# Strong-AI-Lab/ct-vae

Hardware: AMD Instinct MI355X
Metric: images/sec/GPU fwd+bwd, 64×64×3 bs=64; recon+KL vs CPU ref (higher is better)
Workload: dtype f32; 1 GPU; VanillaVAE 64x64x3 train step fwd+loss+bwd+Adam (configs/vae.yaml shapes at the batch BASELINE.json's metric names, bs=64, on one MI355X; BASELINE.json configs[1..4] are the `configs` entries); per_gpu_batch=64, global_batch=64, latent_dim=128, parallelism=single, hipgraph=True, allreduce_overlap=False

## Files before the change

### ct-vae_amd/csrc/pair.hpp

```cpp
#pragma once
#include <functional>
#include <vector>

#include "finish.hpp"
#include "tapgemm.hpp"
#include "wgrad_fast.hpp"

namespace ctvae {

struct PairCtx {
  bool haveA = false, haveB = false;
  long dgrad_wgs = 0;
  int dgrad_chunks = 0;
  TapGemmArgs A;
  unsigned gxA = 0, gyA = 0, gzA = 0;
  double flopsA = 0, bytesA = 0;
  WgradArgs B;
  int lgQw = -1, lgQhw = -1, lgC = -1;
  unsigned gxB = 0, gyB = 0;
  double flopsB = 0, bytesB = 0;
  bool haveSK = false, haveRed = false;
  SplitKJob sk;
  ReduceJob j1, j2;
  int nb1 = 0, nb2 = 0, accumulate = 0;
  double bytesSK = 0, bytesRed = 0;
  bool haveBF = false;
  BnFinJob bf;
  std::vector<std::function<int()>> later;
};

PairCtx*& pair_ctx();
int pair_flush(PairCtx& c, hipStream_t st);
int launch_wgrad_fast_recorded(const PairCtx& c, hipStream_t st);
int launch_finish_recorded(const PairCtx& c, hipStream_t st);
int launch_splitk_recorded(const PairCtx& c, hipStream_t st);
int launch_bn_bwd_finalize_job(const BnFinJob& j, hipStream_t st);

}
```

### ct-vae_amd/csrc/tapgemm_fast.hip

```cpp
#include <type_traits>

#include "prof.hpp"
#include "pair.hpp"
#include "tapgemm.hpp"
#include "wgrad_fast.hpp"

namespace ctvae {

typedef unsigned int u32x4 __attribute__((ext_vector_type(4)));
constexpr unsigned kOOB = 0x80000000u;

__device__ __forceinline__ f32x4 buf_load4(__amdgpu_buffer_rsrc_t r, unsigned voff, unsigned soff) {
  return __builtin_bit_cast(f32x4, __builtin_amdgcn_raw_buffer_load_b128(r, (int)voff, (int)soff, 0));
}
__device__ __forceinline__ float buf_load1(__amdgpu_buffer_rsrc_t r, unsigned voff) {
  return __builtin_bit_cast(float, __builtin_amdgcn_raw_buffer_load_b32(r, (int)voff, 0, 0));
}
__device__ __forceinline__ void buf_store1(__amdgpu_buffer_rsrc_t r, unsigned voff, float v) {
  __builtin_amdgcn_raw_buffer_store_b32(__builtin_bit_cast(unsigned, v), r, (int)voff, 0, 0);
}
__device__ __forceinline__ __amdgpu_buffer_rsrc_t make_rsrc(const void* p, long bytes) {
  return __builtin_amdgcn_make_buffer_rsrc(const_cast<void*>(p), 0, (int)bytes, 0x00020000);
}

// ... 3 lines not shown
__device__ long long g_loop[4 * 8192];
#define LOOPT(var) const long long var = clock64()
#define LOOPACC(i, a, b) loopt_[i] += (b) - (a)
#define LOOPDECL long long loopt_[4] = {0, 0, 0, 0}
#define LOOPOUT do { if (threadIdx.x == 0 && blockIdx.z == 0) for (int q_ = 0; q_ < 4; ++q_) g_loop[((blockIdx.y * gridDim.x + blockIdx.x) & 8191) * 4 + q_] = loopt_[q_]; } while (0)
extern "C" int ctvae_debug_loop_read(long long* out, int n) { return (int)hipMemcpyFromSymbol(out, HIP_SYMBOL(g_loop), (size_t)n * 8); }
extern "C" int ctvae_debug_phase_read(unsigned long long* out, int n) {
  return (int)hipMemcpyFromSymbol(out, HIP_SYMBOL(g_phase), (size_t)n * 8);
}
extern "C" int ctvae_debug_wphase_read(unsigned long long* out, int n) {
  return (int)hipMemcpyFromSymbol(out, HIP_SYMBOL(g_wphase), (size_t)n * 8);
}
#else
#define PHASE(i) do {} while (0)
#define LOOPT(var) do {} while (0)
#define LOOPACC(i, a, b) do {} while (0)
#define LOOPDECL do {} while (0)
#define LOOPOUT do {} while (0)
#endif

template <int WM, int WN, int TM, int TN, bool WT, int PF, bool XF = false, int PD = 1>
__global__ __launch_bounds__(256) void tapgemm_fast_kernel(const TapGemmArgs a) {
  __shared__ __attribute__((aligned(16))) float sAbuf[(PF == 3 ? 2 : 1) * (WM * TM * 32) * LDK];
  __shared__ __attribute__((aligned(16))) float sBbuf[(PF == 3 ? 2 : 1) * (WT ? (WN * TN * 32) * LDK : KC * (WN * TN * 32))];
  __shared__ __attribute__((aligned(16))) int sOut[WM * TM * 32];
  PHASE(0);
  int k_cls_rot, k_mtiles, k_ntiles;
  kernarg_warm_get<sizeof(TapGemmArgs), offsetof(TapGemmArgs, cls_rot), offsetof(TapGemmArgs, mtiles), offsetof(TapGemmArgs, ntiles)>(
      k_cls_rot, k_mtiles, k_ntiles);
  const int vbx = blockIdx.x, vby = blockIdx.y, vbz = blockIdx.z, vgx = k_mtiles * k_ntiles;
#include "tapgemm_fast_body.inc"
}

template <bool XFB, int PDA = 1>
__global__ __launch_bounds__(256) void conv_bwd_pair_kernel(const TapGemmArgs a, const WgradArgs w, int lgQw, int lgQhw, int lgC,
                                                            int nA, int gxA, int gyA, int gxB, int gyB) {
  __shared__ __attribute__((aligned(16))) float sAbuf[2 * 64 * LDK];
  __shared__ __attribute__((aligned(16))) float sBbuf[2 * 64 * LDK];
  __shared__ __attribute__((aligned(16))) int sOut[64];
  __shared__ unsigned sPix[2][MC];
  __shared__ unsigned sMsk[2][MC];
  __shared__ unsigned sOutB[2][MC];
  static_assert(2 * 64 * LDK >= MC * 64, "chunk buffers of the weight-gradient kernel fit");
  constexpr int kOffW = (sizeof(TapGemmArgs) + 7) / 8 * 8, kOffI = kOffW + sizeof(WgradArgs);
  static_assert(alignof(TapGemmArgs) == 8 && alignof(WgradArgs) == 8 && sizeof(WgradArgs) % 8 == 0, "kernel-argument layout");
  int k_nA, k_gxA, k_gyA;
  kernarg_warm_get<kOffI + 8 * 4, kOffI + 12, kOffI + 16, kOffI + 20>(k_nA, k_gxA, k_gyA);
  const int L = blockIdx.x;
  if (L < k_nA) {
    constexpr int WM = 2, WN = 2, TM = 1, TN = 1, PF = 3;
    constexpr bool WT = true, XF = false;
    constexpr int PD = PDA;
    const int vbx = L % k_gxA, vr = L / k_gxA, vby = vr % k_gyA, vbz = vr / k_gyA, vgx = k_gxA;
    const int k_cls_rot = a.cls_rot, k_ntiles = a.ntiles;
#include "tapgemm_fast_body.inc"
  } else {
    const int Lb = L - k_nA;
    wgrad_fast_body<2, 2, 1, 1, XFB>(w, lgQw, lgQhw, lgC, sAbuf, sBbuf, sPix, sMsk, sOutB, Lb % gxB, Lb / gxB, gxB, gyB);
  }
}

template <int WM, int WN, int TM, int TN>
static int launch_fast_cfg(const TapGemmArgs& a, int pf, hipStream_t st) {
  constexpr int BM = WM * TM * 32, BN = WN * TN * 32;
  TapGemmArgs args = a;
  args.mtiles = ceil_div(a.Mc, BM);
  args.ntiles = ceil_div(a.N, BN);
  const bool wt = a.g.wT != 0;
  dim3 grid(args.mtiles * args.ntiles, a.g.ncls, a.splitk > 1 ? a.splitk : 1), block(256);
  for (int c = 0; c < kMaxCls; ++c) args.cls_order[c] = c;
  args.cls_rot = 0;
  if (a.g.ncls == 4) {
    int idx[4] = {0, 1, 2, 3};
    for (int i = 1; i < 4; ++i)
      for (int j = i; j > 0 && a.g.ntaps[idx[j]] < a.g.ntaps[idx[j - 1]]; --j) { const int t = idx[j]; idx[j] = idx[j - 1]; idx[j - 1] = t; }
    const long total = (long)grid.x * grid.y * grid.z;
    if (total <= 1024) {
      args.cls_order[0] = idx[0]; args.cls_order[1] = idx[1]; args.cls_order[2] = idx[3]; args.cls_order[3] = idx[2];
      args.cls_rot = grid.z > 1 ? 1 : 0;
    }
  }
  for (int i = 0; i < kMaxCls; ++i) {
    const int c = args.cls_order[i];
    args.ntaps_l[i] = a.g.ntaps[c];
    for (int t = 0; t < kMaxTaps; ++t) args.taps_l[i][t] = a.g.taps[c][t];
  }
  constexpr bool deep = false;
  char name[160];
  snprintf(name, sizeof name, "tapgemm_fast_kernel<%d,%d,%d,%d,%s,%d%s>", WM, WN, TM, TN, wt ? "true" : "false", pf,
           (!wt && a.xf_scale != nullptr) ? ",true" : (deep ? ",false,4" : ""));
  double macs = 0;
  for (int c = 0; c < a.g.ncls; ++c) macs += (double)a.Mc * a.N * a.g.ntaps[c] * a.g.gC;
  if constexpr (WM == 2 && WN == 2 && TM == 1 && TN == 1) {
    PairCtx* pc = pair_ctx();
    if (pc != nullptr && wt && pf == 3 && !pc->haveA) {
      pc->haveA = true;
      pc->A = args;
      pc->gxA = grid.x; pc->gyA = grid.y; pc->gzA = grid.z;
      pc->flopsA = 2.0 * macs;
      pc->bytesA = 4.0 * ((double)a.g.B * a.g.gH * a.g.gW * a.g.gC + (double)a.g.B * a.g.sH * a.g.sW * a.g.sC);
      return 0;
    }
  }
  if (prof_detailed()) {
    size_t l = strlen(name);
    snprintf(name + l, sizeof name - l, " M=%dx%d N=%d C=%d taps=%d sk=%d", a.g.ncls, a.Mc, a.N, a.g.gC, a.g.ntaps[a.g.ncls - 1],
             a.splitk);
  }
  const double bytes = 4.0 * ((double)a.g.B * a.g.gH * a.g.gW * a.g.gC + (double)a.g.B * a.g.sH * a.g.sW * a.g.sC);
  ProfScope ps(name, st, 2.0 * macs, bytes);
  if (!wt && a.xf_scale != nullptr) {
    if (pf == 3) hipLaunchKernelGGL((tapgemm_fast_kernel<WM, WN, TM, TN, false, 3, true>), grid, block, 0, st, args);
    else hipLaunchKernelGGL((tapgemm_fast_kernel<WM, WN, TM, TN, false, 0, true>), grid, block, 0, st, args);
  } else if (!wt) {
    if (pf == 3) hipLaunchKernelGGL((tapgemm_fast_kernel<WM, WN, TM, TN, false, 3>), grid, block, 0, st, args);
    else hipLaunchKernelGGL((tapgemm_fast_kernel<WM, WN, TM, TN, false, 0>), grid, block, 0, st, args);
  } else {
    if (pf == 3) hipLaunchKernelGGL((tapgemm_fast_kernel<WM, WN, TM, TN, true, 3>), grid, block, 0, st, args);
    else hipLaunchKernelGGL((tapgemm_fast_kernel<WM, WN, TM, TN, true, 0>), grid, block, 0, st, args);
  }
  CTVAE_LAUNCH_CHECK();
  return 0;
}

PairCtx*& pair_ctx() {
  static thread_local PairCtx* ctx = nullptr;
  return ctx;
}

int pair_flush(PairCtx& c, hipStream_t st) {
  if (c.haveA && c.haveB) {
    const unsigned nA = c.gxA * c.gyA * c.gzA, nB = c.gxB * c.gyB;
    ProfScope ps("conv_bwd_pair_kernel", st, c.flopsA + c.flopsB, c.bytesA + c.bytesB);
#define CTVAE_PAIR(XFB_, PD_)                                                                                                  \
  hipLaunchKernelGGL((conv_bwd_pair_kernel<XFB_, PD_>), dim3(nA + nB), dim3(256), 0, st, c.A, c.B, c.lgQw, c.lgQhw, c.lgC, (int)nA, \
                     (int)c.gxA, (int)c.gyA, (int)c.gxB, (int)c.gyB)
    if (c.B.xf_scale != nullptr) CTVAE_PAIR(true, 1);
    else CTVAE_PAIR(false, 1);
#undef CTVAE_PAIR
    CTVAE_LAUNCH_CHECK();
  } else if (c.haveA) {
    ProfScope ps("tapgemm_fast_kernel<2,2,1,1,true,3>", st, c.flopsA, c.bytesA);
    hipLaunchKernelGGL((tapgemm_fast_kernel<2, 2, 1, 1, true, 3>), dim3(c.gxA, c.gyA, c.gzA), dim3(256), 0, st, c.A);
    CTVAE_LAUNCH_CHECK();
  } else if (c.haveB) {
    const int rc = launch_wgrad_fast_recorded(c, st);
    if (rc) return rc;
  }
  if (c.haveRed || (c.haveSK && c.haveBF)) {
    const int rc = launch_finish_recorded(c, st);
    if (rc) return rc;
  } else {
    if (c.haveSK) {
      const int rc = launch_splitk_recorded(c, st);
      if (rc) return rc;
    }
    if (c.haveBF) {
      const int rc = launch_bn_bwd_finalize_job(c.bf, st);
      if (rc) return rc;
    }
  }
  for (auto& f : c.later) {
    const int rc = f();
    if (rc) return rc;
  }
  return 0;
}

int launch_tapgemm_fast(const TapGemmArgs& a, const TapGemmPlan& plan, int pf, hipStream_t st) {
  if (plan.BN == 32) return launch_fast_cfg<4, 1, 1, 1>(a, pf, st);
  if (plan.BM == 128) return launch_fast_cfg<2, 2, 2, 1>(a, pf, st);
  return launch_fast_cfg<2, 2, 1, 1>(a, pf, st);
}

}
```

### ct-vae_amd/csrc/wgrad.hip

```cpp
#include "common.hpp"
#include "prof.hpp"
#include "finish.hpp"
#include "pair.hpp"
#include "wgrad_fast.hpp"

namespace ctvae {


template <int WK, int WN, bool XVEC, bool DVEC>
__global__ __launch_bounds__(256) void wgrad_kernel(const WgradArgs a) {
  kernarg_warm<sizeof(WgradArgs)>();
  constexpr int KT = WK * 32, NT = WN * 32;
  static_assert(WK * WN == 4, "4 waves");
  __shared__ __attribute__((aligned(16))) float sXbuf[MC * KT];
  __shared__ __attribute__((aligned(16))) float sDbuf[MC * NT];
  __shared__ int sRowPix[2][MC];
  __shared__ int sRowYX[2][MC];
  __shared__ int sRowOut[2][MC];

  const ConvGeom& g = a.g;
  const int tid = threadIdx.x, lane = tid & 63, wave = tid >> 6;
  const int wk = wave / WN, wn = wave % WN;
  const int li = lane & 31, lh = lane >> 5;
  int split = blockIdx.y, xtile = blockIdx.x;
  {
    const int T = gridDim.x, L = blockIdx.y * T + blockIdx.x, full = (gridDim.y >> 3) * 8 * T;
    if (L < full) {
      const int grp = L / (8 * T), r = L - grp * 8 * T;
      split = grp * 8 + (r & 7);
      xtile = r >> 3;
    }
  }
  const int ktg = xtile / a.ntiles, nt = xtile - ktg * a.ntiles;
  int cls = 0;
#pragma unroll
  for (int c = 1; c < kMaxCls; ++c)
    if (c < g.ncls && ktg >= a.ktile_start[c]) cls = c;
  const int kt0 = (ktg - a.ktile_start[cls]) * KT;
  const int n0 = nt * NT;
  const int gC = g.gC;
  const int Ktot = g.ntaps[cls] * gC;
  const int N = a.N;

  const int cbeg = split * a.chunks_per_split;
  const int nchunks_all = (a.Mc + MC - 1) / MC;
  int cend = cbeg + a.chunks_per_split;
  if (cend > nchunks_all) cend = nchunks_all;
  const int nch = cend - cbeg;

  auto rowinfo = [&](int c, int buf) {
    if (tid < MC) {
      int m = (cbeg + c) * MC + tid;
      if (m < a.Mc) {
        int b, qy, qx;
        decode_m(g, m, b, qy, qx);
        sRowPix[buf][tid] = (b * g.gH + qy * g.is) * g.gW + qx * g.is;
        sRowYX[buf][tid] = ((qy * g.is) << 16) | (qx * g.is);
        sRowOut[buf][tid] = scatter_pix(g, cls, b, qy, qx);
      } else {
        sRowPix[buf][tid] = -1;
        sRowYX[buf][tid] = 0;
        sRowOut[buf][tid] = -1;
      }
    }
  };

  constexpr int XQ = KT / 4;
  constexpr int X_V = (MC * XQ) / 256;
  constexpr int X_S = (MC * KT) / 256;
  constexpr int DQ = NT / 4;
  constexpr int D_V = (MC * DQ) / 256 > 0 ? (MC * DQ) / 256 : 1;
  constexpr int D_S = (MC * NT) / 256;

  int x_dy = 0, x_dx = 0, x_c = 0;
  bool x_kok = false;
  {
    int kcol = XVEC ? 4 * (tid % XQ) : (tid % KT);
    int k = kt0 + kcol;
    x_kok = k < Ktot;
    int t = x_kok ? k / gC : 0;
    x_c = k - t * gC;
    Tap tp = g.taps[cls][t];
    x_dy = tp.dy;
    x_dx = tp.dx;
  }

  const bool xf_on = XVEC && a.xf_scale != nullptr && x_kok;
  const f32x4 xf_sc = xf_on ? *reinterpret_cast<const f32x4*>(a.xf_scale + x_c) : f32x4{0.f, 0.f, 0.f, 0.f};
  const f32x4 xf_sh = xf_on ? *reinterpret_cast<const f32x4*>(a.xf_shift + x_c) : f32x4{0.f, 0.f, 0.f, 0.f};
  const float xf_ns = a.xf_act == ACT_LRELU ? kLeaky : (a.xf_act == ACT_RELU ? 0.f : 1.f);
  f32x4 rx[XVEC ? X_V : 1];
  [[maybe_unused]] float rx_in[XVEC ? X_V : 1];
  float rxs[XVEC ? 1 : X_S];
  f32x4 rd[DVEC ? D_V : 1];
  [[maybe_unused]] bool rd_ok[DVEC ? D_V : 1];
  float rds[DVEC ? 1 : D_S];

  auto load_chunk = [&](int buf) {
    if constexpr (XVEC) {
      int pixv[X_V], yxv[X_V];
#pragma unroll
      for (int j = 0; j < X_V; ++j) {
        const int r = tid / XQ + (256 / XQ) * j;
        pixv[j] = sRowPix[buf][r];
        yxv[j] = sRowYX[buf][r];
      }
#pragma unroll
      for (int j = 0; j < X_V; ++j) {
        const int iy = (yxv[j] >> 16) + x_dy, ix = (yxv[j] & 0xffff) + x_dx;
        const bool ok = x_kok && pixv[j] >= 0 && (unsigned)iy < (unsigned)g.gH && (unsigned)ix < (unsigned)g.gW;
        const long off = ok ? (long)(pixv[j] + x_dy * g.gW + x_dx) * gC + x_c : 0L;
        rx[j] = *reinterpret_cast<const f32x4*>(a.X + off);
        rx_in[j] = ok ? 1.f : 0.f;
      }
    } else {
#pragma unroll
      for (int j = 0; j < X_S; ++j) {
        int r = tid / KT + (256 / KT) * j;
        int pix = sRowPix[buf][r], yx = sRowYX[buf][r];
        int iy = (yx >> 16) + x_dy, ix = (yx & 0xffff) + x_dx;
        bool ok = x_kok && pix >= 0 && (unsigned)iy < (unsigned)g.gH && (unsigned)ix < (unsigned)g.gW;
        rxs[j] = ok ? a.X[(long)(pix + x_dy * g.gW + x_dx) * gC + x_c] : 0.f;
      }
    }
    if constexpr (DVEC) {
      int spv[D_V];
#pragma unroll
      for (int j = 0; j < D_V; ++j) {
        const int r = (tid + 256 * j) / DQ;
        spv[j] = sRowOut[buf][r < MC ? r : 0];
      }
#pragma unroll
      for (int j = 0; j < D_V; ++j) {
        const int f = tid + 256 * j;
        const int r = f / DQ, nq = f - r * DQ;
        const int n = n0 + 4 * nq;
        const bool ok = r < MC && spv[j] >= 0 && n < N;
        rd[j] = *reinterpret_cast<const f32x4*>(a.dY + (ok ? (long)spv[j] * N + n : 0L));
        rd_ok[j] = ok;
      }
    } else {
#pragma unroll
      for (int j = 0; j < D_S; ++j) {
        int e = tid + 256 * j;
        int r = e / NT, nn = e - r * NT;
        int sp = sRowOut[buf][r];
        int n = n0 + nn;
        rds[j] = (sp >= 0 && n < N) ? a.dY[(long)sp * N + n] : 0.f;
      }
    }
  };

  auto store_chunk = [&]() {
    float* sX = sXbuf;
    float* sD = sDbuf;
    if constexpr (XVEC) {
#pragma unroll
      for (int j = 0; j < X_V; ++j)
        if (rx_in[j] == 0.f) rx[j] = f32x4{0.f, 0.f, 0.f, 0.f};
      if (xf_on) {
#pragma unroll
        for (int j = 0; j < X_V; ++j)
#pragma unroll
          for (int e = 0; e < 4; ++e) {
            const float t = rx[j][e] * xf_sc[e] + xf_sh[e] * rx_in[j];
            rx[j][e] = fmaxf(t, t * xf_ns);
          }
      }
#pragma unroll
      for (int j = 0; j < X_V; ++j) {
        int r = tid / XQ + (256 / XQ) * j;
        *reinterpret_cast<f32x4*>(&sX[r * KT + 4 * (tid % XQ)]) = rx[j];
      }
    } else {
#pragma unroll
      for (int j = 0; j < X_S; ++j) sX[(tid / KT + (256 / KT) * j) * KT + (tid % KT)] = rxs[j];
    }
    if constexpr (DVEC) {
#pragma unroll
      for (int j = 0; j < D_V; ++j) {
        int f = tid + 256 * j;
        int r = f / DQ, nq = f - r * DQ;
        if (r < MC) *reinterpret_cast<f32x4*>(&sD[r * NT + 4 * nq]) = rd_ok[j] ? rd[j] : f32x4{0.f, 0.f, 0.f, 0.f};
      }
    } else {
#pragma unroll
      for (int j = 0; j < D_S; ++j) sD[tid + 256 * j] = rds[j];
    }
  };

  f32x16 acc;
#pragma unroll
  for (int r = 0; r < 16; ++r) acc[r] = 0.f;
  float bsum = 0.f;
  const bool do_bias = (a.pbias != nullptr) && (kt0 == 0) && (tid < NT);

  if (nch > 0) {
    rowinfo(0, 0);
    __syncthreads();
    load_chunk(0);
    if (nch > 1) rowinfo(1, 1);
    store_chunk();
    __syncthreads();
    for (int c = 0; c < nch; ++c) {
      const float* sX = sXbuf;
      const float* sD = sDbuf;
      if (c + 1 < nch) load_chunk((c + 1) & 1);
      if (c + 2 < nch) rowinfo(c + 2, c & 1);
      {
        constexpr int GS = 4, NG = (MC / 2) / GS;
        float fa[2][GS], fb[2][GS];
        auto rdg = [&](int gi, int set) {
#pragma unroll
          for (int q = 0; q < GS; ++q) {
            const int s = gi * GS + q;
            fa[set][q] = sX[(2 * s + lh) * KT + wk * 32 + li];
            fb[set][q] = sD[(2 * s + lh) * NT + wn * 32 + li];
          }
        };
        rdg(0, 0);
#pragma unroll
        for (int gi = 0; gi < NG; ++gi) {
          if (gi + 1 < NG) rdg(gi + 1, (gi + 1) & 1);
#pragma unroll
          for (int q = 0; q < GS; ++q) acc = __builtin_amdgcn_mfma_f32_32x32x2f32(fa[gi & 1][q], fb[gi & 1][q], acc, 0, 0, 0);
#pragma unroll
          for (int q = 0; q < GS; ++q) {
            __builtin_amdgcn_sched_group_barrier(0x008, 1, 0);
            __builtin_amdgcn_sched_group_barrier(0x100, 2, 0);
          }
        }
      }
      if (do_bias) {
#pragma unroll 8
        for (int r = 0; r < MC; ++r) bsum += sD[r * NT + tid];
      }
      __syncthreads();
      if (c + 1 < nch) {
        store_chunk();
        __syncthreads();
      }
    }
  }

  const int col = n0 + wn * 32 + li;
#pragma unroll
  for (int r = 0; r < 16; ++r) {
    int k = kt0 + wk * 32 + 8 * (r >> 2) + 4 * lh + (r & 3);
    if (k < Ktot && col < N) {
      int t = k / gC, c = k - t * gC;
      int wrow = g.taps[cls][t].wtap * (g.wts / g.wCo) + c * (g.wrs / g.wCo);
      a.part[((long)split * a.rows_total + wrow) * N + col] = acc[r];
    }
  }
  if (do_bias && n0 + tid < N) a.pbias[(long)(split * g.ncls + cls) * N + n0 + tid] = bsum;
}

template <int WK, int WN, int TK, int TN, bool XF = false>
__global__ __launch_bounds__(256) void wgrad_fast_kernel(const WgradArgs a, int lgQw, int lgQhw, int lgC) {
  kernarg_warm<sizeof(WgradArgs) + 12>();
  constexpr int KT = WK * TK * 32, NT = WN * TN * 32;
  __shared__ __attribute__((aligned(16))) float sX[MC * KT];
  __shared__ __attribute__((aligned(16))) float sD[MC * NT];
  __shared__ unsigned sPix[2][MC];
  __shared__ unsigned sMsk[2][MC];
  __shared__ unsigned sOutB[2][MC];
  wgrad_fast_body<WK, WN, TK, TN, XF>(a, lgQw, lgQhw, lgC, sX, sD, sPix, sMsk, sOutB, blockIdx.x, blockIdx.y, gridDim.x, gridDim.y);
}


template <typename T>
__device__ __forceinline__ T rzero();
template <>
__device__ __forceinline__ float rzero<float>() { return 0.f; }
template <>
__device__ __forceinline__ f32x4 rzero<f32x4>() { return f32x4{0.f, 0.f, 0.f, 0.f}; }

template <typename T>
__device__ __forceinline__ void reduce_small(const ReduceJob& j, int blk, int accumulate) {
  const long n = j.n / (long)(sizeof(T) / 4), i = (long)blk * 256 + threadIdx.x;
  if (i >= n) return;
  T v = accumulate ? reinterpret_cast<const T*>(j.dst)[i] : rzero<T>();
  for (int s = 0; s < j.S; ++s) v += reinterpret_cast<const T*>(j.part + (long)s * j.stride)[i];
  reinterpret_cast<T*>(j.dst)[i] = v;
}

template <typename T>
__device__ __forceinline__ void reduce_split(const ReduceJob& j, int blk, int accumulate, T (*sm)[64]) {
// ... 319 lines not shown
  if (thin) {
    float *part = nullptr, *pb = nullptr;
    int nw = 0, nb = 0;
    int rc = launch_thin_wgrad(g, X, dY, ws, &part, &pb, &nw, &nb, dbias != nullptr, st, xf);
    if (rc) return rc;
    int taps = 0;
    for (int c = 0; c < g.ncls; ++c) taps += g.ntaps[c];
    const long n = (long)taps * g.gC * g.sC;
    return finish_reduce(part, dW, n, nw, n, pb, dbias, (long)g.sC, nb, (long)g.sC, accumulate, st);
  }
  WgradArgs a{};
  a.g = g;
  a.X = X; a.dY = dY;
  a.Mc = g.B * g.Qh * g.Qw;
  a.N = g.sC;
  if (g.wT != 0 || a.Mc <= 0) return kErrBadArg;
  int taps_total = 0;
  for (int c = 0; c < g.ncls; ++c) taps_total += g.ntaps[c];
  a.rows_total = taps_total * g.gC;
  const bool xvec = (g.gC % 4) == 0, dvec = (a.N % 4) == 0;
  const bool narrow = a.N <= 32;
  bool big = !has_xf && xvec && dvec && (a.N % 128) == 0 && a.Mc >= 8192;
  if (has_xf) { a.xf_scale = xf->scale; a.xf_shift = xf->shift; a.xf_act = xf->act; }
  for (int c = 0; c < g.ncls && big; ++c) big = (g.ntaps[c] * g.gC) % 128 == 0;
  if (big) {
    int tiles128 = 0;
    for (int c = 0; c < g.ncls; ++c) tiles128 += g.ntaps[c] * g.gC / 128;
    tiles128 *= a.N / 128;
    big = tiles128 >= 16 && (long)ceil_div(a.Mc, MC) * tiles128 >= 8L * 1024;
  }
  const int KT = big ? 128 : (narrow ? 128 : 64), NT = big ? 128 : (narrow ? 32 : 64);
  const size_t ws_floats = ws_bytes / sizeof(float);
  const PairCtx* pcw = pair_ctx();
  const bool will_pair = pcw != nullptr && !pcw->haveB && xvec && dvec && !narrow && !big;
  const bool coarse = will_pair && pcw->dgrad_wgs > 0 && pcw->dgrad_wgs < 1024 && pcw->dgrad_chunks >= 12;
  const int S = choose_splits(g, KT, NT, ws_floats, big ? 512 : (coarse ? 768 : 1024));
  if (wgrad_workspace_floats(g, S) > ws_floats) return kErrWorkspace;
  a.S = S;
  const int nchunks = ceil_div(a.Mc, MC);
  a.chunks_per_split = ceil_div(nchunks, S);
  a.part = ws;
  a.pbias = dbias ? ws + (size_t)S * a.rows_total * a.N : nullptr;
  int kt = 0;
  for (int c = 0; c < g.ncls; ++c) {
    a.ktile_start[c] = kt;
    kt += ceil_div(g.ntaps[c] * g.gC, KT);
  }
  a.ktile_start[g.ncls] = kt;
  a.ntiles = ceil_div(a.N, NT);
  dim3 grid(kt * a.ntiles, S), block(256);
  bool recorded = false;
  if (PairCtx* pc = pair_ctx(); pc != nullptr && !pc->haveB && xvec && dvec && !narrow && !big) {
    auto lg2 = [](int v) { int l = 0; while ((1 << l) < v) ++l; return (1 << l) == v ? l : -1; };
    const int lw = lg2(g.Qw), lh2 = lg2(g.Qh);
    pc->haveB = true;
    pc->B = a;
    pc->lgQw = (lw >= 0 && lh2 >= 0) ? lw : -1;
    pc->lgQhw = (lw >= 0 && lh2 >= 0) ? lw + lh2 : -1;
    pc->lgC = lg2(g.gC);
    pc->gxB = grid.x; pc->gyB = grid.y;
    pc->flopsB = 2.0 * (double)a.Mc * a.N * a.rows_total;
    pc->bytesB = 4.0 * ((double)g.B * g.gH * g.gW * g.gC + (double)g.B * g.sH * g.sW * g.sC);
    recorded = true;
  }
  if (!recorded) {
  char name[160];
  if (big) snprintf(name, sizeof name, "wgrad_fast_kernel<2,2,2,2>");
  else if (xvec && dvec && !narrow) snprintf(name, sizeof name, "wgrad_fast_kernel<%d,%d,1,1>", narrow ? 4 : 2, narrow ? 1 : 2);
  else snprintf(name, sizeof name, "wgrad_kernel<%d,%d,%s,%s>", narrow ? 4 : 2, narrow ? 1 : 2, xvec ? "true" : "false",
                dvec ? "true" : "false");
  const double macs = (double)a.Mc * a.N * a.rows_total;
  if (prof_detailed()) {
    size_t l = strlen(name);
    snprintf(name + l, sizeof name - l, " M=%dx%d N=%d rows=%d S=%d", g.ncls, a.Mc, a.N, a.rows_total, S);
  }
  const double bytes = 4.0 * ((double)g.B * g.gH * g.gW * g.gC + (double)g.B * g.sH * g.sW * g.sC);
  ProfScope ps(name, st, 2.0 * macs, bytes);
#define CTVAE_WG(WK_, WN_)                                                                              \
  do {                                                                                                  \
    if (xvec && dvec) hipLaunchKernelGGL((wgrad_kernel<WK_, WN_, true, true>), grid, block, 0, st, a);  \
    else if (!xvec && dvec) hipLaunchKernelGGL((wgrad_kernel<WK_, WN_, false, true>), grid, block, 0, st, a); \
    else if (xvec && !dvec) hipLaunchKernelGGL((wgrad_kernel<WK_, WN_, true, false>), grid, block, 0, st, a); \
    else hipLaunchKernelGGL((wgrad_kernel<WK_, WN_, false, false>), grid, block, 0, st, a);             \
  } while (0)
  if (xvec && dvec && !narrow) {
    auto lg2 = [](int v) { int l = 0; while ((1 << l) < v) ++l; return (1 << l) == v ? l : -1; };
    const int lw = lg2(g.Qw), lh2 = lg2(g.Qh);
    const int lgQw = (lw >= 0 && lh2 >= 0) ? lw : -1, lgQhw = (lw >= 0 && lh2 >= 0) ? lw + lh2 : -1;
    const int lgC = lg2(g.gC);
    if (big) hipLaunchKernelGGL((wgrad_fast_kernel<2, 2, 2, 2>), grid, block, 0, st, a, lgQw, lgQhw, lgC);
    else if (has_xf) hipLaunchKernelGGL((wgrad_fast_kernel<2, 2, 1, 1, true>), grid, block, 0, st, a, lgQw, lgQhw, lgC);
    else hipLaunchKernelGGL((wgrad_fast_kernel<2, 2, 1, 1>), grid, block, 0, st, a, lgQw, lgQhw, lgC);
  } else if (narrow) CTVAE_WG(4, 1);
  else CTVAE_WG(2, 2);
#undef CTVAE_WG
  }
  CTVAE_LAUNCH_CHECK();
  const long n = (long)a.rows_total * a.N;
  const float* part = a.part;
  const float* pbias = a.pbias;
  const int ncls = g.ncls, N_ = a.N;
  return finish_reduce(part, dW, n, S, n, dbias ? pbias : nullptr, dbias, (long)N_, S * ncls, (long)N_, accumulate, st);
}

int launch_finish_recorded(const PairCtx& c, hipStream_t st) {
  const int nsk = c.haveSK ? c.sk.nblk : 0, nbf = c.haveBF ? c.bf.C : 0;
  ProfScope ps(nsk ? "reduce_partials_kernel (+ split-K finish)" : (nbf ? "reduce_partials_kernel (+ BN-backward finalize)" : "reduce_partials_kernel"),
               st, 0.0, c.bytesRed + (nsk ? c.bytesSK : 0.0) + (nbf ? 8.0 * c.bf.nblocks * c.bf.C : 0.0));
  hipLaunchKernelGGL(reduce_partials_kernel, dim3(c.nb1 + c.nb2 + nsk + nbf), dim3(256), 0, st, c.j1, c.j2, c.nb1, c.accumulate,
                     nsk ? c.sk : SplitKJob{}, c.nb1 + c.nb2, nbf ? c.bf : BnFinJob{}, c.nb1 + c.nb2 + nsk);
  CTVAE_LAUNCH_CHECK();
  return 0;
}

int launch_wgrad_fast_recorded(const PairCtx& c, hipStream_t st) {
  ProfScope ps("wgrad_fast_kernel<2,2,1,1>", st, c.flopsB, c.bytesB);
  if (c.B.xf_scale != nullptr)
    hipLaunchKernelGGL((wgrad_fast_kernel<2, 2, 1, 1, true>), dim3(c.gxB, c.gyB), dim3(256), 0, st, c.B, c.lgQw, c.lgQhw, c.lgC);
  else
    hipLaunchKernelGGL((wgrad_fast_kernel<2, 2, 1, 1>), dim3(c.gxB, c.gyB), dim3(256), 0, st, c.B, c.lgQw, c.lgQhw, c.lgC);
  CTVAE_LAUNCH_CHECK();
  return 0;
}

}
```

### ct-vae_amd/csrc/wgrad_fast.hpp

```cpp
#pragma once
#include "common.hpp"

namespace ctvae {

struct WgradArgs {
  ConvGeom g;
  const float* X;
  const float* dY;
  float* part;
  float* pbias;
  int Mc, N, S, chunks_per_split;
  int rows_total;
  int ktile_start[kMaxCls + 1];
  int ntiles;
  const float* xf_scale;
  const float* xf_shift;
  int xf_act;
};

constexpr int MC = 32;

#ifdef CTVAE_PHASE_TIMING
static __device__ unsigned long long g_wphase[8 * 8192];
#define WPHASE(i) do { if (threadIdx.x == 0) g_wphase[((vby * vgx + vbx) & 8191) * 8 + (i)] = wall_clock64(); } while (0)
// ... 209 lines not shown
        bsum += (t0 + t1) + (t2 + t3);
      }
      __syncthreads();
      if (c + 1 < nch) {
        store_chunk();
        __syncthreads();
      }
    }
  }

  WPHASE(3);
#pragma unroll
  for (int i = 0; i < TK; ++i)
#pragma unroll
    for (int j = 0; j < TN; ++j) {
      const int col = n0 + (wn * TN + j) * 32 + li;
#pragma unroll
      for (int q4 = 0; q4 < 4; ++q4) {
        if (wrow0[i][q4] >= 0 && col < N) {
          float* dst = a.part + ((long)split * a.rows_total + wrow0[i][q4]) * N + col;
#pragma unroll
          for (int q = 0; q < 4; ++q) dst[(long)q * wcr * N] = acc[i][j][4 * q4 + q];
        }
      }
    }
  if (do_bias && n0 + tid < N) a.pbias[(long)(split * g.ncls + cls) * N + n0 + tid] = bsum;
#ifdef CTVAE_PHASE_TIMING
  WPHASE(4);
  __builtin_amdgcn_s_waitcnt(0);
  WPHASE(5);
#endif
}

}
```

Before: 87210 images/s.

## Pair narrow-channel wgrad and 4x1 dgrad tiles into the fused backward kernel

Pulls the plain weight-gradient kernel body into a reusable device function so the fused dgrad+wgrad pair kernel can also host the narrow (128x32) wgrad variant. The pair kernel is templated on the dgrad warp layout and the wgrad tile shape, and the narrow case now joins the pair when the dgrad grid is small. The aim is to cut separate launches and fill the GPU better on small-channel backward layers. The cost is extra template instantiations, and shared-memory sizing now depends on tile shape, which could lower occupancy.

```diff
diff --git a/ct-vae_amd/csrc/pair.hpp b/ct-vae_amd/csrc/pair.hpp
--- a/ct-vae_amd/csrc/pair.hpp
+++ b/ct-vae_amd/csrc/pair.hpp
@@ -13,9 +13,11 @@
   long dgrad_wgs = 0;
   int dgrad_chunks = 0;
   TapGemmArgs A;
+  int wmA = 2;
   unsigned gxA = 0, gyA = 0, gzA = 0;
   double flopsA = 0, bytesA = 0;
   WgradArgs B;
+  int wkB = 2;
   int lgQw = -1, lgQhw = -1, lgC = -1;
   unsigned gxB = 0, gyB = 0;
   double flopsB = 0, bytesB = 0;
@@ -31,7 +33,7 @@
 
 PairCtx*& pair_ctx();
 int pair_flush(PairCtx& c, hipStream_t st);
-int launch_wgrad_fast_recorded(const PairCtx& c, hipStream_t st);
+int launch_wgrad_recorded(const PairCtx& c, hipStream_t st);
 int launch_finish_recorded(const PairCtx& c, hipStream_t st);
 int launch_splitk_recorded(const PairCtx& c, hipStream_t st);
 int launch_bn_bwd_finalize_job(const BnFinJob& j, hipStream_t st);
diff --git a/ct-vae_amd/csrc/tapgemm_fast.hip b/ct-vae_amd/csrc/tapgemm_fast.hip
--- a/ct-vae_amd/csrc/tapgemm_fast.hip
+++ b/ct-vae_amd/csrc/tapgemm_fast.hip
@@ -59,23 +59,26 @@
 #include "tapgemm_fast_body.inc"
 }
 
-template <bool XFB, int PDA = 1>
+template <bool XFB, int PDA = 1, int AWM = 2, int BWK = 2>
 __global__ __launch_bounds__(256) void conv_bwd_pair_kernel(const TapGemmArgs a, const WgradArgs w, int lgQw, int lgQhw, int lgC,
                                                             int nA, int gxA, int gyA, int gxB, int gyB) {
-  __shared__ __attribute__((aligned(16))) float sAbuf[2 * 64 * LDK];
-  __shared__ __attribute__((aligned(16))) float sBbuf[2 * 64 * LDK];
-  __shared__ __attribute__((aligned(16))) int sOut[64];
+  static_assert((AWM == 2 || AWM == 4) && (BWK == 2 || BWK == 4), "64 x 64 or 128 x 32 tiles");
+  constexpr int ABM = AWM * 32, ABN = (4 / AWM) * 32;
+  constexpr int BKT = BWK * 32, BNT = (4 / BWK) * 32;
+  __shared__ __attribute__((aligned(16))) float sAbuf[2 * ABM * LDK];
+  __shared__ __attribute__((aligned(16))) float sBbuf[2 * ABN * LDK];
+  __shared__ __attribute__((aligned(16))) int sOut[ABM];
   __shared__ unsigned sPix[2][MC];
   __shared__ unsigned sMsk[2][MC];
   __shared__ unsigned sOutB[2][MC];
-  static_assert(2 * 64 * LDK >= MC * 64, "chunk buffers of the weight-gradient kernel fit");
+  static_assert(2 * ABM * LDK >= MC * BKT && 2 * ABN * LDK >= MC * BNT, "chunk buffers of the weight-gradient kernel fit");
   constexpr int kOffW = (sizeof(TapGemmArgs) + 7) / 8 * 8, kOffI = kOffW + sizeof(WgradArgs);
   static_assert(alignof(TapGemmArgs) == 8 && alignof(WgradArgs) == 8 && sizeof(WgradArgs) % 8 == 0, "kernel-argument layout");
   int k_nA, k_gxA, k_gyA;
   kernarg_warm_get<kOffI + 8 * 4, kOffI + 12, kOffI + 16, kOffI + 20>(k_nA, k_gxA, k_gyA);
   const int L = blockIdx.x;
   if (L < k_nA) {
-    constexpr int WM = 2, WN = 2, TM = 1, TN = 1, PF = 3;
+    constexpr int WM = AWM, WN = 4 / AWM, TM = 1, TN = 1, PF = 3;
     constexpr bool WT = true, XF = false;
     constexpr int PD = PDA;
     const int vbx = L % k_gxA, vr = L / k_gxA, vby = vr % k_gyA, vbz = vr / k_gyA, vgx = k_gxA;
@@ -83,7 +86,12 @@
 #include "tapgemm_fast_body.inc"
   } else {
     const int Lb = L - k_nA;
-    wgrad_fast_body<2, 2, 1, 1, XFB>(w, lgQw, lgQhw, lgC, sAbuf, sBbuf, sPix, sMsk, sOutB, Lb % gxB, Lb / gxB, gxB, gyB);
+    if constexpr (BWK == 4) {
+      wgrad_plain_body<4, 1, true, true>(w, sAbuf, sBbuf, reinterpret_cast<int(*)[MC]>(sPix), reinterpret_cast<int(*)[MC]>(sMsk),
+                                         reinterpret_cast<int(*)[MC]>(sOutB), Lb % gxB, Lb / gxB, gxB, gyB);
+    } else {
+      wgrad_fast_body<2, 2, 1, 1, XFB>(w, lgQw, lgQhw, lgC, sAbuf, sBbuf, sPix, sMsk, sOutB, Lb % gxB, Lb / gxB, gxB, gyB);
+    }
   }
 }
 
@@ -118,10 +126,11 @@
            (!wt && a.xf_scale != nullptr) ? ",true" : (deep ? ",false,4" : ""));
   double macs = 0;
   for (int c = 0; c < a.g.ncls; ++c) macs += (double)a.Mc * a.N * a.g.ntaps[c] * a.g.gC;
-  if constexpr (WM == 2 && WN == 2 && TM == 1 && TN == 1) {
+  if constexpr (TM == 1 && TN == 1) {
     PairCtx* pc = pair_ctx();
     if (pc != nullptr && wt && pf == 3 && !pc->haveA) {
       pc->haveA = true;
+      pc->wmA = WM;
       pc->A = args;
       pc->gxA = grid.x; pc->gyA = grid.y; pc->gzA = grid.z;
       pc->flopsA = 2.0 * macs;
@@ -159,19 +168,30 @@
   if (c.haveA && c.haveB) {
     const unsigned nA = c.gxA * c.gyA * c.gzA, nB = c.gxB * c.gyB;
     ProfScope ps("conv_bwd_pair_kernel", st, c.flopsA + c.flopsB, c.bytesA + c.bytesB);
-#define CTVAE_PAIR(XFB_, PD_)                                                                                                  \
-  hipLaunchKernelGGL((conv_bwd_pair_kernel<XFB_, PD_>), dim3(nA + nB), dim3(256), 0, st, c.A, c.B, c.lgQw, c.lgQhw, c.lgC, (int)nA, \
-                     (int)c.gxA, (int)c.gyA, (int)c.gxB, (int)c.gyB)
-    if (c.B.xf_scale != nullptr) CTVAE_PAIR(true, 1);
-    else CTVAE_PAIR(false, 1);
+#define CTVAE_PAIR(XFB_, AWM_, BWK_)                                                                                                  \
+  hipLaunchKernelGGL((conv_bwd_pair_kernel<XFB_, 1, AWM_, BWK_>), dim3(nA + nB), dim3(256), 0, st, c.A, c.B, c.lgQw, c.lgQhw, c.lgC, \
+                     (int)nA, (int)c.gxA, (int)c.gyA, (int)c.gxB, (int)c.gyB)
+    const bool xfb = c.B.xf_scale != nullptr;
+    if (c.wkB == 4) {
+      if (c.wmA == 4) CTVAE_PAIR(false, 4, 4);
+      else CTVAE_PAIR(false, 2, 4);
+    } else if (c.wmA == 4) {
+      if (xfb) CTVAE_PAIR(true, 4, 2);
+      else CTVAE_PAIR(false, 4, 2);
+    } else if (xfb) {
+      CTVAE_PAIR(true, 2, 2);
+    } else {
+      CTVAE_PAIR(false, 2, 2);
+    }
 #undef CTVAE_PAIR
     CTVAE_LAUNCH_CHECK();
   } else if (c.haveA) {
-    ProfScope ps("tapgemm_fast_kernel<2,2,1,1,true,3>", st, c.flopsA, c.bytesA);
-    hipLaunchKernelGGL((tapgemm_fast_kernel<2, 2, 1, 1, true, 3>), dim3(c.gxA, c.gyA, c.gzA), dim3(256), 0, st, c.A);
+    ProfScope ps(c.wmA == 4 ? "tapgemm_fast_kernel<4,1,1,1,true,3>" : "tapgemm_fast_kernel<2,2,1,1,true,3>", st, c.flopsA, c.bytesA);
+    if (c.wmA == 4) hipLaunchKernelGGL((tapgemm_fast_kernel<4, 1, 1, 1, true, 3>), dim3(c.gxA, c.gyA, c.gzA), dim3(256), 0, st, c.A);
+    else hipLaunchKernelGGL((tapgemm_fast_kernel<2, 2, 1, 1, true, 3>), dim3(c.gxA, c.gyA, c.gzA), dim3(256), 0, st, c.A);
     CTVAE_LAUNCH_CHECK();
   } else if (c.haveB) {
-    const int rc = launch_wgrad_fast_recorded(c, st);
+    const int rc = launch_wgrad_recorded(c, st);
     if (rc) return rc;
   }
   if (c.haveRed || (c.haveSK && c.haveBF)) {
diff --git a/ct-vae_amd/csrc/wgrad.hip b/ct-vae_amd/csrc/wgrad.hip
--- a/ct-vae_amd/csrc/wgrad.hip
+++ b/ct-vae_amd/csrc/wgrad.hip
@@ -10,250 +10,12 @@
 template <int WK, int WN, bool XVEC, bool DVEC>
 __global__ __launch_bounds__(256) void wgrad_kernel(const WgradArgs a) {
   kernarg_warm<sizeof(WgradArgs)>();
-  constexpr int KT = WK * 32, NT = WN * 32;
-  static_assert(WK * WN == 4, "4 waves");
-  __shared__ __attribute__((aligned(16))) float sXbuf[MC * KT];
-  __shared__ __attribute__((aligned(16))) float sDbuf[MC * NT];
+  __shared__ __attribute__((aligned(16))) float sXbuf[MC * WK * 32];
+  __shared__ __attribute__((aligned(16))) float sDbuf[MC * WN * 32];
   __shared__ int sRowPix[2][MC];
   __shared__ int sRowYX[2][MC];
   __shared__ int sRowOut[2][MC];
-
-  const ConvGeom& g = a.g;
-  const int tid = threadIdx.x, lane = tid & 63, wave = tid >> 6;
-  const int wk = wave / WN, wn = wave % WN;
-  const int li = lane & 31, lh = lane >> 5;
-  int split = blockIdx.y, xtile = blockIdx.x;
-  {
-    const int T = gridDim.x, L = blockIdx.y * T + blockIdx.x, full = (gridDim.y >> 3) * 8 * T;
-    if (L < full) {
-      const int grp = L / (8 * T), r = L - grp * 8 * T;
-      split = grp * 8 + (r & 7);
-      xtile = r >> 3;
-    }
-  }
-  const int ktg = xtile / a.ntiles, nt = xtile - ktg * a.ntiles;
-  int cls = 0;
-#pragma unroll
-  for (int c = 1; c < kMaxCls; ++c)
-    if (c < g.ncls && ktg >= a.ktile_start[c]) cls = c;
-  const int kt0 = (ktg - a.ktile_start[cls]) * KT;
-  const int n0 = nt * NT;
-  const int gC = g.gC;
-  const int Ktot = g.ntaps[cls] * gC;
-  const int N = a.N;
-
-  const int cbeg = split * a.chunks_per_split;
-  const int nchunks_all = (a.Mc + MC - 1) / MC;
-  int cend = cbeg + a.chunks_per_split;
-  if (cend > nchunks_all) cend = nchunks_all;
-  const int nch = cend - cbeg;
-
-  auto rowinfo = [&](int c, int buf) {
-    if (tid < MC) {
-      int m = (cbeg + c) * MC + tid;
-      if (m < a.Mc) {
-        int b, qy, qx;
-        decode_m(g, m, b, qy, qx);
-        sRowPix[buf][tid] = (b * g.gH + qy * g.is) * g.gW + qx * g.is;
-        sRowYX[buf][tid] = ((qy * g.is) << 16) | (qx * g.is);
-        sRowOut[buf][tid] = scatter_pix(g, cls, b, qy, qx);
-      } else {
-        sRowPix[buf][tid] = -1;
-        sRowYX[buf][tid] = 0;
-        sRowOut[buf][tid] = -1;
-      }
-    }
-  };
-
-  constexpr int XQ = KT / 4;
-  constexpr int X_V = (MC * XQ) / 256;
-  constexpr int X_S = (MC * KT) / 256;
-  constexpr int DQ = NT / 4;
-  constexpr int D_V = (MC * DQ) / 256 > 0 ? (MC * DQ) / 256 : 1;
-  constexpr int D_S = (MC * NT) / 256;
-
-  int x_dy = 0, x_dx = 0, x_c = 0;
-  bool x_kok = false;
-  {
-    int kcol = XVEC ? 4 * (tid % XQ) : (tid % KT);
-    int k = kt0 + kcol;
-    x_kok = k < Ktot;
-    int t = x_kok ? k / gC : 0;
-    x_c = k - t * gC;
-    Tap tp = g.taps[cls][t];
-    x_dy = tp.dy;
-    x_dx = tp.dx;
-  }
-
-  const bool xf_on = XVEC && a.xf_scale != nullptr && x_kok;
-  const f32x4 xf_sc = xf_on ? *reinterpret_cast<const f32x4*>(a.xf_scale + x_c) : f32x4{0.f, 0.f, 0.f, 0.f};
-  const f32x4 xf_sh = xf_on ? *reinterpret_cast<const f32x4*>(a.xf_shift + x_c) : f32x4{0.f, 0.f, 0.f, 0.f};
-  const float xf_ns = a.xf_act == ACT_LRELU ? kLeaky : (a.xf_act == ACT_RELU ? 0.f : 1.f);
-  f32x4 rx[XVEC ? X_V : 1];
-  [[maybe_unused]] float rx_in[XVEC ? X_V : 1];
-  float rxs[XVEC ? 1 : X_S];
-  f32x4 rd[DVEC ? D_V : 1];
-  [[maybe_unused]] bool rd_ok[DVEC ? D_V : 1];
-  float rds[DVEC ? 1 : D_S];
-
-  auto load_chunk = [&](int buf) {
-    if constexpr (XVEC) {
-      int pixv[X_V], yxv[X_V];
-#pragma unroll
-      for (int j = 0; j < X_V; ++j) {
-        const int r = tid / XQ + (256 / XQ) * j;
-        pixv[j] = sRowPix[buf][r];
-        yxv[j] = sRowYX[buf][r];
-      }
-#pragma unroll
-      for (int j = 0; j < X_V; ++j) {
-        const int iy = (yxv[j] >> 16) + x_dy, ix = (yxv[j] & 0xffff) + x_dx;
-        const bool ok = x_kok && pixv[j] >= 0 && (unsigned)iy < (unsigned)g.gH && (unsigned)ix < (unsigned)g.gW;
-        const long off = ok ? (long)(pixv[j] + x_dy * g.gW + x_dx) * gC + x_c : 0L;
-        rx[j] = *reinterpret_cast<const f32x4*>(a.X + off);
-        rx_in[j] = ok ? 1.f : 0.f;
-      }
-    } else {
-#pragma unroll
-      for (int j = 0; j < X_S; ++j) {
-        int r = tid / KT + (256 / KT) * j;
-        int pix = sRowPix[buf][r], yx = sRowYX[buf][r];
-        int iy = (yx >> 16) + x_dy, ix = (yx & 0xffff) + x_dx;
-        bool ok = x_kok && pix >= 0 && (unsigned)iy < (unsigned)g.gH && (unsigned)ix < (unsigned)g.gW;
-        rxs[j] = ok ? a.X[(long)(pix + x_dy * g.gW + x_dx) * gC + x_c] : 0.f;
-      }
-    }
-    if constexpr (DVEC) {
-      int spv[D_V];
-#pragma unroll
-      for (int j = 0; j < D_V; ++j) {
-        const int r = (tid + 256 * j) / DQ;
-        spv[j] = sRowOut[buf][r < MC ? r : 0];
-      }
-#pragma unroll
-      for (int j = 0; j < D_V; ++j) {
-        const int f = tid + 256 * j;
-        const int r = f / DQ, nq = f - r * DQ;
-        const int n = n0 + 4 * nq;
-        const bool ok = r < MC && spv[j] >= 0 && n < N;
-        rd[j] = *reinterpret_cast<const f32x4*>(a.dY + (ok ? (long)spv[j] * N + n : 0L));
-        rd_ok[j] = ok;
-      }
-    } else {
-#pragma unroll
-      for (int j = 0; j < D_S; ++j) {
-        int e = tid + 256 * j;
-        int r = e / NT, nn = e - r * NT;
-        int sp = sRowOut[buf][r];
-        int n = n0 + nn;
-        rds[j] = (sp >= 0 && n < N) ? a.dY[(long)sp * N + n] : 0.f;
-      }
-    }
-  };
-
-  auto store_chunk = [&]() {
-    float* sX = sXbuf;
-    float* sD = sDbuf;
-    if constexpr (XVEC) {
-#pragma unroll
-      for (int j = 0; j < X_V; ++j)
-        if (rx_in[j] == 0.f) rx[j] = f32x4{0.f, 0.f, 0.f, 0.f};
-      if (xf_on) {
-#pragma unroll
-        for (int j = 0; j < X_V; ++j)
-#pragma unroll
-          for (int e = 0; e < 4; ++e) {
-            const float t = rx[j][e] * xf_sc[e] + xf_sh[e] * rx_in[j];
-            rx[j][e] = fmaxf(t, t * xf_ns);
-          }
-      }
-#pragma unroll
-      for (int j = 0; j < X_V; ++j) {
-        int r = tid / XQ + (256 / XQ) * j;
-        *reinterpret_cast<f32x4*>(&sX[r * KT + 4 * (tid % XQ)]) = rx[j];
-      }
-    } else {
-#pragma unroll
-      for (int j = 0; j < X_S; ++j) sX[(tid / KT + (256 / KT) * j) * KT + (tid % KT)] = rxs[j];
-    }
-    if constexpr (DVEC) {
-#pragma unroll
-      for (int j = 0; j < D_V; ++j) {
-        int f = tid + 256 * j;
-        int r = f / DQ, nq = f - r * DQ;
-        if (r < MC) *reinterpret_cast<f32x4*>(&sD[r * NT + 4 * nq]) = rd_ok[j] ? rd[j] : f32x4{0.f, 0.f, 0.f, 0.f};
-      }
-    } else {
-#pragma unroll
-      for (int j = 0; j < D_S; ++j) sD[tid + 256 * j] = rds[j];
-    }
-  };
-
-  f32x16 acc;
-#pragma unroll
-  for (int r = 0; r < 16; ++r) acc[r] = 0.f;
-  float bsum = 0.f;
-  const bool do_bias = (a.pbias != nullptr) && (kt0 == 0) && (tid < NT);
-
-  if (nch > 0) {
-    rowinfo(0, 0);
-    __syncthreads();
-    load_chunk(0);
-    if (nch > 1) rowinfo(1, 1);
-    store_chunk();
-    __syncthreads();
-    for (int c = 0; c < nch; ++c) {
-      const float* sX = sXbuf;
-      const float* sD = sDbuf;
-      if (c + 1 < nch) load_chunk((c + 1) & 1);
-      if (c + 2 < nch) rowinfo(c + 2, c & 1);
-      {
-        constexpr int GS = 4, NG = (MC / 2) / GS;
-        float fa[2][GS], fb[2][GS];
-        auto rdg = [&](int gi, int set) {
-#pragma unroll
-          for (int q = 0; q < GS; ++q) {
-            const int s = gi * GS + q;
-            fa[set][q] = sX[(2 * s + lh) * KT + wk * 32 + li];
-            fb[set][q] = sD[(2 * s + lh) * NT + wn * 32 + li];
-          }
-        };
-        rdg(0, 0);
-#pragma unroll
-        for (int gi = 0; gi < NG; ++gi) {
-          if (gi + 1 < NG) rdg(gi + 1, (gi + 1) & 1);
-#pragma unroll
-          for (int q = 0; q < GS; ++q) acc = __builtin_amdgcn_mfma_f32_32x32x2f32(fa[gi & 1][q], fb[gi & 1][q], acc, 0, 0, 0);
-#pragma unroll
-          for (int q = 0; q < GS; ++q) {
-            __builtin_amdgcn_sched_group_barrier(0x008, 1, 0);
-            __builtin_amdgcn_sched_group_barrier(0x100, 2, 0);
-          }
-        }
-      }
-      if (do_bias) {
-#pragma unroll 8
-        for (int r = 0; r < MC; ++r) bsum += sD[r * NT + tid];
-      }
-      __syncthreads();
-      if (c + 1 < nch) {
-        store_chunk();
-        __syncthreads();
-      }
-    }
-  }
-
-  const int col = n0 + wn * 32 + li;
-#pragma unroll
-  for (int r = 0; r < 16; ++r) {
-    int k = kt0 + wk * 32 + 8 * (r >> 2) + 4 * lh + (r & 3);
-    if (k < Ktot && col < N) {
-      int t = k / gC, c = k - t * gC;
-      int wrow = g.taps[cls][t].wtap * (g.wts / g.wCo) + c * (g.wrs / g.wCo);
-      a.part[((long)split * a.rows_total + wrow) * N + col] = acc[r];
-    }
-  }
-  if (do_bias && n0 + tid < N) a.pbias[(long)(split * g.ncls + cls) * N + n0 + tid] = bsum;
+  wgrad_plain_body<WK, WN, XVEC, DVEC>(a, sXbuf, sDbuf, sRowPix, sRowYX, sRowOut, blockIdx.x, blockIdx.y, gridDim.x, gridDim.y);
 }
 
 template <int WK, int WN, int TK, int TN, bool XF = false>
@@ -639,7 +401,8 @@
   const int KT = big ? 128 : (narrow ? 128 : 64), NT = big ? 128 : (narrow ? 32 : 64);
   const size_t ws_floats = ws_bytes / sizeof(float);
   const PairCtx* pcw = pair_ctx();
-  const bool will_pair = pcw != nullptr && !pcw->haveB && xvec && dvec && !narrow && !big;
+  const bool will_pair = pcw != nullptr && !pcw->haveB && xvec && dvec && !big &&
+                         (!narrow || (pcw->dgrad_wgs > 0 && pcw->dgrad_wgs < 1024));
   const bool coarse = will_pair && pcw->dgrad_wgs > 0 && pcw->dgrad_wgs < 1024 && pcw->dgrad_chunks >= 12;
   const int S = choose_splits(g, KT, NT, ws_floats, big ? 512 : (coarse ? 768 : 1024));
   if (wgrad_workspace_floats(g, S) > ws_floats) return kErrWorkspace;
@@ -657,10 +420,11 @@
   a.ntiles = ceil_div(a.N, NT);
   dim3 grid(kt * a.ntiles, S), block(256);
   bool recorded = false;
-  if (PairCtx* pc = pair_ctx(); pc != nullptr && !pc->haveB && xvec && dvec && !narrow && !big) {
+  if (PairCtx* pc = pair_ctx(); will_pair) {
     auto lg2 = [](int v) { int l = 0; while ((1 << l) < v) ++l; return (1 << l) == v ? l : -1; };
     const int lw = lg2(g.Qw), lh2 = lg2(g.Qh);
     pc->haveB = true;
+    pc->wkB = narrow ? 4 : 2;
     pc->B = a;
     pc->lgQw = (lw >= 0 && lh2 >= 0) ? lw : -1;
     pc->lgQhw = (lw >= 0 && lh2 >= 0) ? lw + lh2 : -1;
@@ -720,7 +484,13 @@
   return 0;
 }
 
-int launch_wgrad_fast_recorded(const PairCtx& c, hipStream_t st) {
+int launch_wgrad_recorded(const PairCtx& c, hipStream_t st) {
+  if (c.wkB == 4) {
+    ProfScope ps("wgrad_kernel<4,1,true,true>", st, c.flopsB, c.bytesB);
+    hipLaunchKernelGGL((wgrad_kernel<4, 1, true, true>), dim3(c.gxB, c.gyB), dim3(256), 0, st, c.B);
+    CTVAE_LAUNCH_CHECK();
+    return 0;
+  }
   ProfScope ps("wgrad_fast_kernel<2,2,1,1>", st, c.flopsB, c.bytesB);
   if (c.B.xf_scale != nullptr)
     hipLaunchKernelGGL((wgrad_fast_kernel<2, 2, 1, 1, true>), dim3(c.gxB, c.gyB), dim3(256), 0, st, c.B, c.lgQw, c.lgQhw, c.lgC);
diff --git a/ct-vae_amd/csrc/wgrad_fast.hpp b/ct-vae_amd/csrc/wgrad_fast.hpp
--- a/ct-vae_amd/csrc/wgrad_fast.hpp
+++ b/ct-vae_amd/csrc/wgrad_fast.hpp
@@ -265,4 +265,248 @@
 #endif
 }
 
+template <int WK, int WN, bool XVEC, bool DVEC>
+__device__ __forceinline__ void wgrad_plain_body(const WgradArgs& a, float* sXbuf, float* sDbuf, int (*sRowPix)[MC],
+                                                 int (*sRowYX)[MC], int (*sRowOut)[MC], int vbx, int vby, int vgx, int vgy) {
+  constexpr int KT = WK * 32, NT = WN * 32;
+  static_assert(WK * WN == 4, "4 waves");
+
+  const ConvGeom& g = a.g;
+  const int tid = threadIdx.x, lane = tid & 63, wave = tid >> 6;
+  const int wk = wave / WN, wn = wave % WN;
+  const int li = lane & 31, lh = lane >> 5;
+  int split = vby, xtile = vbx;
+  {
+    const int T = vgx, L = vby * T + vbx, full = (vgy >> 3) * 8 * T;
+    if (L < full) {
+      const int grp = L / (8 * T), r = L - grp * 8 * T;
+      split = grp * 8 + (r & 7);
+      xtile = r >> 3;
+    }
+  }
+  const int ktg = xtile / a.ntiles, nt = xtile - ktg * a.ntiles;
+  int cls = 0;
+#pragma unroll
+  for (int c = 1; c < kMaxCls; ++c)
+    if (c < g.ncls && ktg >= a.ktile_start[c]) cls = c;
+  const int kt0 = (ktg - a.ktile_start[cls]) * KT;
+  const int n0 = nt * NT;
+  const int gC = g.gC;
+  const int Ktot = g.ntaps[cls] * gC;
+  const int N = a.N;
+
+  const int cbeg = split * a.chunks_per_split;
+  const int nchunks_all = (a.Mc + MC - 1) / MC;
+  int cend = cbeg + a.chunks_per_split;
+  if (cend > nchunks_all) cend = nchunks_all;
+  const int nch = cend - cbeg;
+
+  auto rowinfo = [&](int c, int buf) {
+    if (tid < MC) {
+      int m = (cbeg + c) * MC + tid;
+      if (m < a.Mc) {
+        int b, qy, qx;
+        decode_m(g, m, b, qy, qx);
+        sRowPix[buf][tid] = (b * g.gH + qy * g.is) * g.gW + qx * g.is;
+        sRowYX[buf][tid] = ((qy * g.is) << 16) | (qx * g.is);
+        sRowOut[buf][tid] = scatter_pix(g, cls, b, qy, qx);
+      } else {
+        sRowPix[buf][tid] = -1;
+        sRowYX[buf][tid] = 0;
+        sRowOut[buf][tid] = -1;
+      }
+    }
+  };
+
+  constexpr int XQ = KT / 4;
+  constexpr int X_V = (MC * XQ) / 256;
+  constexpr int X_S = (MC * KT) / 256;
+  constexpr int DQ = NT / 4;
+  constexpr int D_V = (MC * DQ) / 256 > 0 ? (MC * DQ) / 256 : 1;
+  constexpr int D_S = (MC * NT) / 256;
+
+  int x_dy = 0, x_dx = 0, x_c = 0;
+  bool x_kok = false;
+  {
+    int kcol = XVEC ? 4 * (tid % XQ) : (tid % KT);
+    int k = kt0 + kcol;
+    x_kok = k < Ktot;
+    int t = x_kok ? k / gC : 0;
+    x_c = k - t * gC;
+    Tap tp = g.taps[cls][t];
+    x_dy = tp.dy;
+    x_dx = tp.dx;
+  }
+
+  const bool xf_on = XVEC && a.xf_scale != nullptr && x_kok;
+  const f32x4 xf_sc = xf_on ? *reinterpret_cast<const f32x4*>(a.xf_scale + x_c) : f32x4{0.f, 0.f, 0.f, 0.f};
+  const f32x4 xf_sh = xf_on ? *reinterpret_cast<const f32x4*>(a.xf_shift + x_c) : f32x4{0.f, 0.f, 0.f, 0.f};
+  const float xf_ns = a.xf_act == ACT_LRELU ? kLeaky : (a.xf_act == ACT_RELU ? 0.f : 1.f);
+  f32x4 rx[XVEC ? X_V : 1];
+  [[maybe_unused]] float rx_in[XVEC ? X_V : 1];
+  float rxs[XVEC ? 1 : X_S];
+  f32x4 rd[DVEC ? D_V : 1];
+  [[maybe_unused]] bool rd_ok[DVEC ? D_V : 1];
+  float rds[DVEC ? 1 : D_S];
+
+  auto load_chunk = [&](int buf) {
+    if constexpr (XVEC) {
+      int pixv[X_V], yxv[X_V];
+#pragma unroll
+      for (int j = 0; j < X_V; ++j) {
+        const int r = tid / XQ + (256 / XQ) * j;
+        pixv[j] = sRowPix[buf][r];
+        yxv[j] = sRowYX[buf][r];
+      }
+#pragma unroll
+      for (int j = 0; j < X_V; ++j) {
+        const int iy = (yxv[j] >> 16) + x_dy, ix = (yxv[j] & 0xffff) + x_dx;
+        const bool ok = x_kok && pixv[j] >= 0 && (unsigned)iy < (unsigned)g.gH && (unsigned)ix < (unsigned)g.gW;
+        const long off = ok ? (long)(pixv[j] + x_dy * g.gW + x_dx) * gC + x_c : 0L;
+        rx[j] = *reinterpret_cast<const f32x4*>(a.X + off);
+        rx_in[j] = ok ? 1.f : 0.f;
+      }
+    } else {
+#pragma unroll
+      for (int j = 0; j < X_S; ++j) {
+        int r = tid / KT + (256 / KT) * j;
+        int pix = sRowPix[buf][r], yx = sRowYX[buf][r];
+        int iy = (yx >> 16) + x_dy, ix = (yx & 0xffff) + x_dx;
+        bool ok = x_kok && pix >= 0 && (unsigned)iy < (unsigned)g.gH && (unsigned)ix < (unsigned)g.gW;
+        rxs[j] = ok ? a.X[(long)(pix + x_dy * g.gW + x_dx) * gC + x_c] : 0.f;
+      }
+    }
+    if constexpr (DVEC) {
+      int spv[D_V];
+#pragma unroll
+      for (int j = 0; j < D_V; ++j) {
+        const int r = (tid + 256 * j) / DQ;
+        spv[j] = sRowOut[buf][r < MC ? r : 0];
+      }
+#pragma unroll
+      for (int j = 0; j < D_V; ++j) {
+        const int f = tid + 256 * j;
+        const int r = f / DQ, nq = f - r * DQ;
+        const int n = n0 + 4 * nq;
+        const bool ok = r < MC && spv[j] >= 0 && n < N;
+        rd[j] = *reinterpret_cast<const f32x4*>(a.dY + (ok ? (long)spv[j] * N + n : 0L));
+        rd_ok[j] = ok;
+      }
+    } else {
+#pragma unroll
+      for (int j = 0; j < D_S; ++j) {
+        int e = tid + 256 * j;
+        int r = e / NT, nn = e - r * NT;
+        int sp = sRowOut[buf][r];
+        int n = n0 + nn;
+        rds[j] = (sp >= 0 && n < N) ? a.dY[(long)sp * N + n] : 0.f;
+      }
+    }
+  };
+
+  auto store_chunk = [&]() {
+    float* sX = sXbuf;
+    float* sD = sDbuf;
+    if constexpr (XVEC) {
+#pragma unroll
+      for (int j = 0; j < X_V; ++j)
+        if (rx_in[j] == 0.f) rx[j] = f32x4{0.f, 0.f, 0.f, 0.f};
+      if (xf_on) {
+#pragma unroll
+        for (int j = 0; j < X_V; ++j)
+#pragma unroll
+          for (int e = 0; e < 4; ++e) {
+            const float t = rx[j][e] * xf_sc[e] + xf_sh[e] * rx_in[j];
+            rx[j][e] = fmaxf(t, t * xf_ns);
+          }
+      }
+#pragma unroll
+      for (int j = 0; j < X_V; ++j) {
+        int r = tid / XQ + (256 / XQ) * j;
+        *reinterpret_cast<f32x4*>(&sX[r * KT + 4 * (tid % XQ)]) = rx[j];
+      }
+    } else {
+#pragma unroll
+      for (int j = 0; j < X_S; ++j) sX[(tid / KT + (256 / KT) * j) * KT + (tid % KT)] = rxs[j];
+    }
+    if constexpr (DVEC) {
+#pragma unroll
+      for (int j = 0; j < D_V; ++j) {
+        int f = tid + 256 * j;
+        int r = f / DQ, nq = f - r * DQ;
+        if (r < MC) *reinterpret_cast<f32x4*>(&sD[r * NT + 4 * nq]) = rd_ok[j] ? rd[j] : f32x4{0.f, 0.f, 0.f, 0.f};
+      }
+    } else {
+#pragma unroll
+      for (int j = 0; j < D_S; ++j) sD[tid + 256 * j] = rds[j];
+    }
+  };
+
+  f32x16 acc;
+#pragma unroll
+  for (int r = 0; r < 16; ++r) acc[r] = 0.f;
+  float bsum = 0.f;
+  const bool do_bias = (a.pbias != nullptr) && (kt0 == 0) && (tid < NT);
+
+  if (nch > 0) {
+    rowinfo(0, 0);
+    __syncthreads();
+    load_chunk(0);
+    if (nch > 1) rowinfo(1, 1);
+    store_chunk();
+    __syncthreads();
+    for (int c = 0; c < nch; ++c) {
+      const float* sX = sXbuf;
+      const float* sD = sDbuf;
+      if (c + 1 < nch) load_chunk((c + 1) & 1);
+      if (c + 2 < nch) rowinfo(c + 2, c & 1);
+      {
+        constexpr int GS = 4, NG = (MC / 2) / GS;
+        float fa[2][GS], fb[2][GS];
+        auto rdg = [&](int gi, int set) {
+#pragma unroll
+          for (int q = 0; q < GS; ++q) {
+            const int s = gi * GS + q;
+            fa[set][q] = sX[(2 * s + lh) * KT + wk * 32 + li];
+            fb[set][q] = sD[(2 * s + lh) * NT + wn * 32 + li];
+          }
+        };
+        rdg(0, 0);
+#pragma unroll
+        for (int gi = 0; gi < NG; ++gi) {
+          if (gi + 1 < NG) rdg(gi + 1, (gi + 1) & 1);
+#pragma unroll
+          for (int q = 0; q < GS; ++q) acc = __builtin_amdgcn_mfma_f32_32x32x2f32(fa[gi & 1][q], fb[gi & 1][q], acc, 0, 0, 0);
+#pragma unroll
+          for (int q = 0; q < GS; ++q) {
+            __builtin_amdgcn_sched_group_barrier(0x008, 1, 0);
+            __builtin_amdgcn_sched_group_barrier(0x100, 2, 0);
+          }
+        }
+      }
+      if (do_bias) {
+#pragma unroll 8
+        for (int r = 0; r < MC; ++r) bsum += sD[r * NT + tid];
+      }
+      __syncthreads();
+      if (c + 1 < nch) {
+        store_chunk();
+        __syncthreads();
+      }
+    }
+  }
+
+  const int col = n0 + wn * 32 + li;
+#pragma unroll
+  for (int r = 0; r < 16; ++r) {
+    int k = kt0 + wk * 32 + 8 * (r >> 2) + 4 * lh + (r & 3);
+    if (k < Ktot && col < N) {
+      int t = k / gC, c = k - t * gC;
+      int wrow = g.taps[cls][t].wtap * (g.wts / g.wCo) + c * (g.wrs / g.wCo);
+      a.part[((long)split * a.rows_total + wrow) * N + col] = acc[r];
+    }
+  }
+  if (do_bias && n0 + tid < N) a.pbias[(long)(split * g.ncls + cls) * N + n0 + tid] = bsum;
 }
+
+}
```

Result: faster. 89050 images/s (median of 6 runs) (+2.1%).
